# Deam0on/deepEMIA

Hardware: NVIDIA B200
Metric: instances_per_sec (higher is better)
Workload: dtype f32

## Files before the change

__graft_entry__.py:

```python
import os
import subprocess
import sys

ROOT = os.path.dirname(os.path.abspath(__file__))
CSRC = os.path.join(ROOT, "deepemia_b200", "csrc")
NVCC_FLAGS = ["-O3", "-lineinfo", "-fmad=false", "-std=c++17", "-gencode", "arch=compute_100a,code=sm_100a", "-shared",
              "-Xcompiler", "-fPIC"]


def _newer(target, sources):
    if not os.path.exists(target):
        return True
    t = os.path.getmtime(target)
    return any(os.path.getmtime(s) > t for s in sources)


def _sources():
    out = []
    for d, _, files in os.walk(CSRC):
        out += [os.path.join(d, f) for f in files if f.endswith((".cu", ".cuh", ".h"))]
    out.append(os.path.join(ROOT, "include", "emia.h"))
    return out


# ... 2 lines not shown
    if force or _newer(lib, _sources()):
        nvcc = os.environ.get("NVCC", "/usr/local/cuda/bin/nvcc")
        cmd = [nvcc] + NVCC_FLAGS + [os.path.join(CSRC, "emia_kernels.cu"), "-o", lib]
        subprocess.check_call(cmd, cwd=CSRC)
    hs_dir = os.path.join(ROOT, "tests", "hostsim")
    hs = os.path.join(hs_dir, "libemia_hostsim.so")
    if force or _newer(hs, _sources() + [os.path.join(hs_dir, "hostsim.cpp")]):
        subprocess.check_call(["g++", "-O2", "-ffp-contract=off", "-fPIC", "-shared", "-x", "c++", "hostsim.cpp", "-o", hs],
                              cwd=hs_dir)
    hs_rle = os.path.join(hs_dir, "libemia_hostsim_rle.so")
    if force or _newer(hs_rle, _sources() + [os.path.join(hs_dir, "hostsim_rle.cpp")]):
        subprocess.check_call(["g++", "-O2", "-ffp-contract=off", "-fPIC", "-shared", "-x", "c++", "hostsim_rle.cpp", "-o", hs_rle],
                              cwd=hs_dir)
    hs_text = os.path.join(hs_dir, "libemia_hostsim_text.so")
    if force or _newer(hs_text, _sources() + [os.path.join(hs_dir, "hostsim_text.cpp")]):
        subprocess.check_call(["g++", "-O2", "-ffp-contract=off", "-fPIC", "-shared", "-pthread", "-x", "c++", "hostsim_text.cpp", "-o",
                               hs_text], cwd=hs_dir)
    hs_shape = os.path.join(hs_dir, "libemia_hostsim_shape.so")
    if force or _newer(hs_shape, _sources() + [os.path.join(hs_dir, "hostsim_shape.cpp")]):
        subprocess.check_call(["g++", "-O2", "-ffp-contract=off", "-fPIC", "-shared", "-x", "c++", "hostsim_shape.cpp", "-o", hs_shape],
                              cwd=hs_dir)
    hs_nb = os.path.join(hs_dir, "libemia_hostsim_neighbour.so")
    if force or _newer(hs_nb, _sources() + [os.path.join(hs_dir, "hostsim_neighbour.cpp")]):
        subprocess.check_call(["g++", "-O2", "-ffp-contract=off", "-fPIC", "-shared", "-x", "c++", "hostsim_neighbour.cpp", "-o", hs_nb],
                              cwd=hs_dir)
    hs_trace = os.path.join(hs_dir, "libemia_hostsim_trace.so")
    if force or _newer(hs_trace, _sources() + [os.path.join(hs_dir, "hostsim_trace.cpp")]):
        subprocess.check_call(["g++", "-O2", "-ffp-contract=off", "-fPIC", "-shared", "-x", "c++", "hostsim_trace.cpp", "-o", hs_trace],
                              cwd=hs_dir)
    hs_coco = os.path.join(hs_dir, "libemia_hostsim_coco.so")
    if force or _newer(hs_coco, _sources() + [os.path.join(hs_dir, "hostsim_coco.cpp")]):
        subprocess.check_call(["g++", "-O2", "-ffp-contract=off", "-fPIC", "-shared", "-x", "c++", "hostsim_coco.cpp", "-o", hs_coco],
                              cwd=hs_dir)
    demo_dir = os.path.join(ROOT, "tests", "abi_demo")
    demo = os.path.join(demo_dir, "abi_demo")
    if force or _newer(demo, [os.path.join(demo_dir, "abi_demo.cpp"), os.path.join(ROOT, "include", "emia.h"), lib]):
        nvcc = os.environ.get("NVCC", "/usr/local/cuda/bin/nvcc")
        subprocess.check_call([nvcc, "-O2", "-std=c++17", "abi_demo.cpp", "-o", demo, "-L" + os.path.join(ROOT, "deepemia_b200"), "-lemia",
                               "-Xlinker", "-rpath", "-Xlinker", os.path.join("$ORIGIN", "..", "..", "deepemia_b200")], cwd=demo_dir)
    if ROOT not in sys.path:
        sys.path.insert(0, ROOT)
    import deepemia_b200
    from deepemia_b200 import _lib
    _lib.load()


def smoke():
    if ROOT not in sys.path:
        sys.path.insert(0, ROOT)
    import numpy as np
    import torch
    from deepemia_b200 import engine, synthetic as syn
    from oracle import pipeline
    dev = torch.device("cuda:0")
    H = W = 256
    probs, boxes, scores, classes = syn.synthetic_heads(42, 40, H, W, duplicate_frac=0.3, rmin=6, rmax=20, margin=20)
    t = [torch.as_tensor(a, device=dev) for a in (probs, boxes, scores, classes)]
    iset, kept, meas = engine.run_tiles(*t, [0, len(probs)], H, W, um_pix=0.5, rules=syn.POLYHIPES_RULES, frames=True)
    torch.cuda.synchronize()
    final, rows, _ = pipeline.run_tile(probs, boxes, scores, classes, H, W, um_pix=0.5, rules=syn.POLYHIPES_RULES)
    got = kept.to_lists()[0]
    assert got == final, (got, final)
    vals = [r[:12] for _, rr in meas.rows_to_host()[0] for r in rr if r[15] == 1.0]
    assert len(vals) == len(rows)
    for g, r in zip(vals, rows):
        np.testing.assert_allclose(g, np.array([float(v) for v in r[3:15]]), rtol=1e-5, atol=0)
# ... 8 lines not shown
```

deepemia_b200/_lib.py:

```python
import ctypes
import os

_HERE = os.path.dirname(os.path.abspath(__file__))
LIB_PATH = os.environ.get("EMIA_LIB_PATH") or os.path.join(_HERE, "libemia.so")

c_void_p, c_int, c_int64, c_float, c_double, c_size_t = (ctypes.c_void_p, ctypes.c_int, ctypes.c_int64, ctypes.c_float,
                                                         ctypes.c_double, ctypes.c_size_t)


class EmiaError(RuntimeError):
    pass


_SIGNATURES = {
    "emia_version": (c_int, []),
    "emia_last_error": (ctypes.c_char_p, []),
    "emia_scan_workspace_bytes": (c_size_t, [c_int64]),
    "emia_exclusive_scan_i64": (c_int, [c_void_p, c_int64, c_void_p, c_size_t, c_void_p]),
    "emia_paste_plan": (c_int, [c_void_p, c_int64, c_float, c_float, c_int, c_int, c_void_p, c_void_p, c_void_p]),
    "emia_paste_threshold_bitpack": (c_int, [c_void_p, c_void_p, c_void_p, c_void_p, c_int64, c_float, c_float, c_int, c_int,
                                             c_void_p, c_int64, c_int, c_void_p, c_void_p, c_void_p, c_int, c_void_p, c_void_p]),
    "emia_mask_bbox": (c_int, [c_void_p, c_int64, c_int, c_int, c_void_p, c_void_p, c_void_p, c_void_p, c_void_p]),
    "emia_mask_pack": (c_int, [c_void_p, c_int64, c_int, c_int, c_void_p, c_void_p, c_void_p, c_void_p]),
    "emia_mask_unpack": (c_int, [c_void_p, c_void_p, c_void_p, c_void_p, c_int64, c_int, c_int, c_void_p, c_void_p]),
    "emia_contour_count": (c_int, [c_void_p, c_void_p, c_void_p, c_int64, c_void_p, c_void_p, c_void_p, c_void_p, c_void_p]),
    "emia_contour_measure": (c_int, [c_void_p, c_void_p, c_void_p, c_int64, c_void_p, c_void_p, c_void_p, c_void_p, c_double,
                                     c_double, c_void_p, c_void_p, c_void_p, c_void_p, c_void_p, c_void_p, c_void_p]),
    "emia_contour_store": (c_int, [c_void_p, c_void_p, c_void_p, c_int64, c_void_p, c_void_p, c_void_p, c_void_p, c_void_p, c_void_p,
                                   c_void_p]),
    "emia_contour_trace_plan": (c_int, [c_void_p, c_int64, c_void_p, c_void_p]),
    "emia_contour_trace_slab": (c_int, [c_void_p, c_void_p, c_void_p, c_int64, c_void_p, c_void_p, c_int, c_void_p, c_void_p, c_void_p,
                                        c_void_p, c_void_p, c_void_p, c_void_p, c_void_p]),
    "emia_list_measure_plan": (c_int, [c_void_p, c_int, c_int, c_void_p, c_void_p, c_void_p, c_void_p, c_void_p, c_void_p, c_void_p,
                                       c_void_p]),
    "emia_contour_measure_list": (c_int, [c_int64, c_void_p, c_void_p, c_void_p, c_void_p, c_void_p, c_void_p, c_int, c_double, c_double,
                                          c_void_p, c_void_p, c_void_p, c_void_p, c_void_p, c_void_p, c_void_p]),
    "emia_list_measure_order": (c_int, [c_int64, c_void_p, c_void_p, c_void_p, c_void_p, c_int, c_void_p, c_void_p, c_void_p]),
    "emia_contour_shape_list": (c_int, [c_int64, c_void_p, c_void_p, c_void_p, c_void_p, c_void_p, c_void_p, c_int, c_double, c_void_p,
                                        c_void_p, c_void_p, c_void_p, c_void_p, c_void_p]),
    "emia_contour_measure_stored": (c_int, [c_void_p, c_int64, c_void_p, c_void_p, c_void_p, c_int, c_void_p, c_double, c_double,
                                            c_void_p, c_void_p, c_void_p, c_void_p, c_void_p, c_void_p]),
    "emia_group_workspace_bytes": (c_size_t, [c_void_p, c_int]),
    "emia_dedup_smart": (c_int, [c_void_p, c_void_p, c_void_p, c_void_p, c_void_p, c_void_p, c_void_p, c_void_p, c_void_p,
                                 c_void_p, c_int, c_int, c_int, c_void_p, c_void_p, c_double, c_double, c_void_p, c_void_p, c_void_p,
                                 c_size_t, c_void_p]),
    "emia_dedup_inorder": (c_int, [c_void_p, c_void_p, c_void_p, c_void_p, c_void_p, c_void_p, c_int, c_int, c_int, c_void_p, c_void_p,
                                   c_double, c_void_p, c_void_p, c_void_p, c_size_t, c_void_p]),
    "emia_dedup_sorted": (c_int, [c_void_p, c_void_p, c_void_p, c_void_p, c_void_p, c_void_p, c_void_p, c_int, c_int, c_int, c_void_p,
                                  c_void_p, c_double, c_void_p, c_void_p, c_void_p, c_size_t, c_void_p]),
    "emia_overlap_rules": (c_int, [c_void_p, c_void_p, c_void_p, c_void_p, c_void_p, c_void_p, c_void_p, c_void_p, c_int, c_int, c_int,
                                   c_void_p, c_void_p, c_void_p, c_void_p, c_int, c_void_p, c_void_p, c_void_p, c_size_t,
                                   c_void_p]),
    "emia_containment_rules": (c_int, [c_void_p, c_void_p, c_void_p, c_void_p, c_void_p, c_void_p, c_void_p, c_int, c_int, c_int,
                                       c_void_p, c_void_p, c_void_p, c_void_p, c_int, c_double, c_void_p, c_void_p, c_void_p,
# ... 103 lines not shown
```

deepemia_b200/csrc/core/emia_paste.cuh:

```cuda
#pragma once
#include "emia_common.cuh"

#define EMIA_MASK_SIDE 28

struct EmiaPasteBox {
    float x0, y0, x1, y1;
    int rx0, ry0, rx1, ry1;
    int valid;
};

EMIA_HD float emia_clampf(float v, float lo, float hi) { return v < lo ? lo : (v > hi ? hi : v); }

EMIA_HD EmiaPasteBox emia_paste_prepare(float bx0, float by0, float bx1, float by1, float scale_x, float scale_y, int W, int H) {
    EmiaPasteBox b;
    b.x0 = emia_clampf(bx0 * scale_x, 0.f, (float)W);
    b.x1 = emia_clampf(bx1 * scale_x, 0.f, (float)W);
    b.y0 = emia_clampf(by0 * scale_y, 0.f, (float)H);
    b.y1 = emia_clampf(by1 * scale_y, 0.f, (float)H);
    b.valid = ((b.x1 - b.x0) > 0.f) && ((b.y1 - b.y0) > 0.f);
    b.rx0 = emia_max((int)floorf(b.x0) - 1, 0);
    b.ry0 = emia_max((int)floorf(b.y0) - 1, 0);
    b.rx1 = emia_min((int)ceilf(b.x1) + 1, W);
    b.ry1 = emia_min((int)ceilf(b.y1) + 1, H);
    if (!b.valid) { b.rx0 = b.ry0 = b.rx1 = b.ry1 = 0; }
// ... 8 lines not shown

EMIA_HD EmiaAxisTap emia_paste_axis(int p, float lo, float hi) {
    const float c = (float)p + 0.5f;
    const float t = (c - lo) / (hi - lo);
    const float g = t * 2.f - 1.f;
    const float ix = emia_fmaf(g + 1.f, (float)EMIA_MASK_SIDE * 0.5f, -0.5f);
    const float fl = floorf(ix);
    EmiaAxisTap a;
    a.i0 = (int)fl;
    a.w1 = ix - fl;
    a.w0 = 1.f - a.w1;
    return a;
}

EMIA_HD float emia_paste_tap(const float* prob, int x, int y) {
    return ((unsigned)x < (unsigned)EMIA_MASK_SIDE && (unsigned)y < (unsigned)EMIA_MASK_SIDE) ? prob[y * EMIA_MASK_SIDE + x] : 0.f;
}

EMIA_HD float emia_paste_sample(const float* prob, const EmiaAxisTap& ax, const EmiaAxisTap& ay) {
    const float nw = ay.w0 * ax.w0;
    const float ne = ay.w0 * ax.w1;
    const float sw = ay.w1 * ax.w0;
    const float se = ay.w1 * ax.w1;
    const float v_nw = emia_paste_tap(prob, ax.i0, ay.i0);
    const float v_ne = emia_paste_tap(prob, ax.i0 + 1, ay.i0);
    const float v_sw = emia_paste_tap(prob, ax.i0, ay.i0 + 1);
    const float v_se = emia_paste_tap(prob, ax.i0 + 1, ay.i0 + 1);
    float acc = v_nw * nw;
    acc = emia_fmaf(v_ne, ne, acc);
    acc = emia_fmaf(v_sw, sw, acc);
    acc = emia_fmaf(v_se, se, acc);
    return acc;
}
```

deepemia_b200/csrc/emia_kernels.cu:

```cuda
#include <cuda_runtime.h>
#include <cuda_fp16.h>
#include <stdio.h>
#include <stdlib.h>
#include <string.h>
#include <algorithm>
#include <type_traits>
#include "../../include/emia.h"
#include "core/emia_common.cuh"
#include "core/emia_contour.cuh"
#include "core/emia_hull.cuh"
#include "core/emia_ellipse.cuh"
#include "core/emia_measure.cuh"
#include "core/emia_paste.cuh"
#include "core/emia_nms.cuh"
#include "core/emia_moments.cuh"
#include "core/emia_rle.cuh"
#include "core/emia_text.cuh"
#include "core/emia_shape.cuh"
#include "core/emia_neighbour.cuh"
#include "core/emia_coco.cuh"

static thread_local char g_err[512] = "";
static int emia_fail(int code, const char* fmt, const char* detail) {
    snprintf(g_err, sizeof(g_err), fmt, detail);
// ... 472 lines not shown
        }
        __syncthreads();
        (void)piece_rows_bytes;
    }
    if (tid == 0) asm volatile("cp.async.bulk.wait_group 0;" ::: "memory");
}

#define EMIA_P2_PAD_STRIDE 36
#define EMIA_P2_PAD_ROWS 32
#define EMIA_P2_BAND_ROWS 128
#define EMIA_P2_MAX_COLS 2112
#ifndef EMIA_P2_MIN_CTAS
#define EMIA_P2_MIN_CTAS 4
#endif

__device__ __forceinline__ void emia_st256_zero(void* p) {
    asm volatile("st.global.v4.b64 [%0], {%1, %1, %1, %1};" ::"l"(p), "l"(0ull) : "memory");
}
__device__ __forceinline__ void emia_st256(void* p, uint4 a, uint4 b) {
    asm volatile("st.global.v4.b64 [%0], {%1, %2, %3, %4};" ::"l"(p), "l"(((unsigned long long)a.y << 32) | a.x),
                 "l"(((unsigned long long)a.w << 32) | a.z), "l"(((unsigned long long)b.y << 32) | b.x),
                 "l"(((unsigned long long)b.w << 32) | b.z)
                 : "memory");
}
__device__ __forceinline__ void emia_cp_async16(void* sdst, const void* gsrc) {
    asm volatile("cp.async.cg.shared.global [%0], [%1], 16;" ::"r"((uint32_t)__cvta_generic_to_shared(sdst)), "l"(gsrc) : "memory");
}
__device__ __forceinline__ int emia_clampi(int v, int lo, int hi) { return v < lo ? lo : (v > hi ? hi : v); }

template <bool kHalf>
__global__ void __launch_bounds__(EMIA_PASTE_THREADS, EMIA_P2_MIN_CTAS) k_paste_v2(
    const void* __restrict__ probs_raw, const float4* __restrict__ boxes, const emia_inst_meta* __restrict__ meta,
    const int64_t* __restrict__ crop_off, int64_t n, float sx, float sy, int H, int W, uint32_t* __restrict__ frames,
    int64_t frame_slots, int pitch_words, uint32_t* __restrict__ crops, int32_t* __restrict__ bbox, int32_t* __restrict__ area,
    const int32_t* __restrict__ abort_flag) {
    if (abort_flag && *abort_flag) return;
    __shared__ __align__(16) float s_pp2[2][EMIA_P2_PAD_ROWS * EMIA_P2_PAD_STRIDE];
    __shared__ __align__(16) __half s_half2[2][kHalf ? EMIA_MASK_SIDE * EMIA_MASK_SIDE : 8];
    const float* probs = (const float*)probs_raw;
    const __half* probs_h = (const __half*)probs_raw;
    __shared__ __align__(32) uint32_t s_tile[EMIA_PASTE_TILE_WORDS];
    __shared__ int2 s_ctap[EMIA_P2_MAX_COLS];
    __shared__ int2 s_rtap[EMIA_P2_BAND_ROWS];
    __shared__ int s_red[5];

    const int tid = threadIdx.x;
    const int lane = tid & 31;
    const int warp = tid >> 5;
    const int nwarps = EMIA_PASTE_THREADS / 32;
    const int cpr = pitch_words >> 3;
    for (int k = tid; k < 2 * EMIA_P2_PAD_ROWS * EMIA_P2_PAD_STRIDE; k += EMIA_PASTE_THREADS) (&s_pp2[0][0])[k] = 0.f;
    __syncthreads();
    auto issue = [&](int64_t q, bool q_live, int b) {
        if (q_live) {
            if (kHalf) {
                if (tid < (EMIA_MASK_SIDE * EMIA_MASK_SIDE) / 8)
                    emia_cp_async16(&s_half2[b][tid * 8], probs_h + q * (EMIA_MASK_SIDE * EMIA_MASK_SIDE) + tid * 8);
            } else if (tid < EMIA_MASK_SIDE * 7) {
                const int r = tid / 7, c7 = tid - r * 7;
                emia_cp_async16(&s_pp2[b][(r + 2) * EMIA_P2_PAD_STRIDE + 4 + c7 * 4],
                                probs + q * (EMIA_MASK_SIDE * EMIA_MASK_SIDE) + r * EMIA_MASK_SIDE + c7 * 4);
            }
        }
        asm volatile("cp.async.commit_group;" ::: "memory");
    };
    emia_inst_meta m_next;
    float4 bx_next = make_float4(0.f, 0.f, 0.f, 0.f);
    m_next.valid = 0; m_next.ch = m_next.cw = 0;
    if ((int64_t)blockIdx.x < n) { m_next = meta[blockIdx.x]; bx_next = boxes[blockIdx.x]; }
    issue(blockIdx.x, (int64_t)blockIdx.x < n && m_next.valid && m_next.ch > 0 && m_next.cw > 0, 0);
    int buf = 0;

    for (int64_t inst = blockIdx.x; inst < n; inst += gridDim.x) {
        const emia_inst_meta m = m_next;
        const float4 bx = bx_next;
        float* s_pp = s_pp2[buf];
        const __half* s_half = s_half2[buf];
        const EmiaPasteBox pb = emia_paste_prepare(bx.x, bx.y, bx.z, bx.w, sx, sy, W, H);
        const bool live = m.valid && m.ch > 0 && m.cw > 0;
        if (tid < 5) s_red[tid] = (tid == 0) ? 0 : ((tid == 1 || tid == 2) ? 0x7fffffff : -1);
        const int cc0 = live ? (m.wc0 >> 3) : 0;
        const int cc1 = live ? ((m.wc0 + m.cw - 1) >> 3) : -1;
        unsigned char* frame = nullptr;
        if (frames) {
            frame = (unsigned char*)(frames + (size_t)(inst % frame_slots) * (size_t)H * (size_t)pitch_words);
            const int total = H * cpr;
            const int top = live ? m.ry0 * cpr : total;
            const int bot0 = live ? (m.ry0 + m.ch) * cpr : total;
            for (int q = tid; q < top; q += EMIA_PASTE_THREADS) emia_st256_zero(frame + (size_t)q * 32);
            for (int q = bot0 + tid; q < total; q += EMIA_PASTE_THREADS) emia_st256_zero(frame + (size_t)q * 32);
            if (live && cc1 - cc0 + 1 < cpr) {
                for (int r = tid; r < m.ch; r += EMIA_PASTE_THREADS) {
                    unsigned char* row = frame + (size_t)(m.ry0 + r) * cpr * 32;
                    for (int c = 0; c < cc0; ++c) emia_st256_zero(row + c * 32);
                    for (int c = cc1 + 1; c < cpr; ++c) emia_st256_zero(row + c * 32);
                }
            }
        }
        {
            const int64_t nx = inst + gridDim.x;
            bool nlive = false;
            if (nx < n) { m_next = meta[nx]; bx_next = boxes[nx]; nlive = m_next.valid && m_next.ch > 0 && m_next.cw > 0; }
            issue(nx, nlive, buf ^ 1);
        }
        if (live) {
            const int ncols = m.cw * 32;
            for (int k = tid; k < ncols; k += EMIA_PASTE_THREADS) {
                const int x = m.wc0 * 32 + k;
                const EmiaAxisTap a = emia_paste_axis(x, pb.x0, pb.x1);
                const int i0 = (x >= m.rx0 && x < m.rx1) ? emia_clampi(a.i0, -2, EMIA_MASK_SIDE) : -2;
                s_ctap[k] = make_int2(i0 + 4, __float_as_int(a.w1));
            }
        }
        asm volatile("cp.async.wait_group 1;" ::: "memory");
        __syncthreads();
        if (kHalf) {
            if (live)
                for (int k = tid; k < EMIA_MASK_SIDE * EMIA_MASK_SIDE; k += EMIA_PASTE_THREADS) {
                    const int r = k / EMIA_MASK_SIDE, c = k - r * EMIA_MASK_SIDE;
                    s_pp[(r + 2) * EMIA_P2_PAD_STRIDE + 4 + c] = __half2float(s_half[k]);
                }
            __syncthreads();
        }
        if (live) {
            const int span_chunks = cc1 - cc0 + 1;
            const int span_words = span_chunks * 8;
            const int woff = m.wc0 - cc0 * 8;
            const int rows_per_band = emia_min(EMIA_P2_BAND_ROWS, emia_max(1, EMIA_PASTE_TILE_WORDS / span_words));
// ... 15 lines not shown
                    const float xw0 = 1.f - xw1, yw0 = 1.f - yw1;
                    const float* t = &s_pp[rt.x + ct.x];
                    const float nw = yw0 * xw0;
                    const float ne = yw0 * xw1;
                    const float sw = yw1 * xw0;
                    const float se = yw1 * xw1;
                    float acc = t[0] * nw;
                    acc = emia_fmaf(t[1], ne, acc);
                    acc = emia_fmaf(t[EMIA_P2_PAD_STRIDE], sw, acc);
                    acc = emia_fmaf(t[EMIA_P2_PAD_STRIDE + 1], se, acc);
                    const uint32_t word = __ballot_sync(0xffffffffu, acc >= 0.5f);
                    if (lane == 0) s_tile[r * span_words + woff + c] = word;
                    r += step_r; c += step_c;
                    if (c >= m.cw) { c -= m.cw; ++r; }
                }
                __syncthreads();
                {
                    int rr = tid / m.cw, cc = tid - rr * m.cw;
                    const int sr = EMIA_PASTE_THREADS / m.cw, scw = EMIA_PASTE_THREADS - sr * m.cw;
                    while (rr < nr) {
                        const uint32_t word = s_tile[rr * span_words + woff + cc];
                        crop[(size_t)(r0 + rr) * m.cw + cc] = word;
                        if (word) {
                            const int y = m.ry0 + r0 + rr;
                            l_area += __popc(word);
                            l_ymin = min(l_ymin, y); l_ymax = max(l_ymax, y);
                            l_xmin = min(l_xmin, (m.wc0 + cc) * 32 + (__ffs((int)word) - 1));
                            l_xmax = max(l_xmax, (m.wc0 + cc) * 32 + (31 - __clz((int)word)));
                        }
                        rr += sr; cc += scw;
                        if (cc >= m.cw) { cc -= m.cw; ++rr; }
                    }
                }
                if (frames) {
                    const uint4* s4 = (const uint4*)s_tile;
                    int rr = tid / span_chunks, cc = tid - rr * span_chunks;
                    const int sr = EMIA_PASTE_THREADS / span_chunks, sc = EMIA_PASTE_THREADS - sr * span_chunks;
                    while (rr < nr) {
                        const int si = (rr * span_chunks + cc) * 2;
                        emia_st256(frame + ((size_t)(m.ry0 + r0 + rr) * cpr + cc0 + cc) * 32, s4[si], s4[si + 1]);
                        rr += sr; cc += sc;
                        if (cc >= span_chunks) { cc -= span_chunks; ++rr; }
                    }
                }
                __syncthreads();
            }
            for (int o = 16; o > 0; o >>= 1) {
                l_area += __shfl_xor_sync(0xffffffffu, l_area, o);
                l_ymin = min(l_ymin, __shfl_xor_sync(0xffffffffu, l_ymin, o)); l_xmin = min(l_xmin, __shfl_xor_sync(0xffffffffu, l_xmin, o));
                l_ymax = max(l_ymax, __shfl_xor_sync(0xffffffffu, l_ymax, o)); l_xmax = max(l_xmax, __shfl_xor_sync(0xffffffffu, l_xmax, o));
            }
            if (lane == 0 && l_area) {
                atomicAdd(&s_red[0], l_area);
                atomicMin(&s_red[1], l_ymin); atomicMin(&s_red[2], l_xmin);
                atomicMax(&s_red[3], l_ymax); atomicMax(&s_red[4], l_xmax);
            }
            __syncthreads();
        }
        if (tid == 0) {
            const int a = live ? s_red[0] : 0;
            area[inst] = a;
            ((int4*)bbox)[inst] = a > 0 ? make_int4(s_red[1], s_red[2], s_red[3], s_red[4]) : make_int4(-1, -1, -1, -1);
        }
        __syncthreads();
        buf ^= 1;
    }
    asm volatile("cp.async.wait_group 0;" ::: "memory");
}

extern "C" int emia_paste_threshold_bitpack(const float* probs, const float* boxes, const emia_inst_meta* meta,
                                            const int64_t* crop_off, int64_t n, float scale_x, float scale_y, int H,
                                            int W, uint32_t* frames, int64_t frame_slots, int pitch_words,
                                            uint32_t* crops, int32_t* bbox, int32_t* area, int variant_and_grid,
                                            const int32_t* abort_flag, void* stream) {
    const int variant = variant_and_grid & 0xff;
    const int ctas_req = (variant_and_grid >> 8) & 0xff;
    const bool probs_f16 = (variant_and_grid >> 16) & 1;
    if (n < 0 || H <= 0 || W <= 0) return emia_fail(EMIA_ERR_BAD_ARG, "emia_paste_threshold_bitpack: %s", "bad shape");
    if (n == 0) return EMIA_OK;
    if (!probs || !boxes || !meta || !crop_off || !crops || !bbox || !area)
        return emia_fail(EMIA_ERR_BAD_ARG, "emia_paste_threshold_bitpack: %s", "null pointer");
    if (frames) {
        if (pitch_words * 32 < W || (pitch_words & 3) || frame_slots <= 0)
            return emia_fail(EMIA_ERR_BAD_ARG, "emia_paste_threshold_bitpack: %s", "pitch_words must be a multiple of 4 covering W; frame_slots > 0");
        if (((uintptr_t)frames & 15) != 0) return emia_fail(EMIA_ERR_BAD_ARG, "emia_paste_threshold_bitpack: %s", "frames must be 16-byte aligned");
    }
    const int max_cols = ((W + 31) / 32 + 1) * 32;
    cudaStream_t st = (cudaStream_t)stream;
    const int sms = emia_num_sms();
    if (variant == 2 && max_cols <= EMIA_P2_MAX_COLS && ((uintptr_t)probs & 15) == 0 &&
        (!frames || ((pitch_words & 7) == 0 && ((uintptr_t)frames & 31) == 0))) {
        const int64_t per_sm = ctas_req ? ctas_req : 32;
        const unsigned grid = (unsigned)(n < (int64_t)sms * per_sm ? n : (int64_t)sms * per_sm);
        if (probs_f16)
            k_paste_v2<true><<<grid, EMIA_PASTE_THREADS, 0, st>>>(probs, (const float4*)boxes, meta, crop_off, n, scale_x, scale_y, H, W, frames,
                                                                  frames ? frame_slots : 1, pitch_words, crops, bbox, area, abort_flag);
        else
            k_paste_v2<false><<<grid, EMIA_PASTE_THREADS, 0, st>>>(probs, (const float4*)boxes, meta, crop_off, n, scale_x, scale_y, H, W, frames,
                                                                   frames ? frame_slots : 1, pitch_words, crops, bbox, area, abort_flag);
        return emia_check_launch("emia_paste_threshold_bitpack (v2) launch: %s");
    }
    if (probs_f16) return emia_fail(EMIA_ERR_UNSUPPORTED, "emia_paste_threshold_bitpack: %s", "fp16 probabilities need variant 2 (W <= 2048, 32-byte frame rows)");
    if (variant == 1 && frames) {
        if (pitch_words * 4 > EMIA_BULK_BYTES) return emia_fail(EMIA_ERR_UNSUPPORTED, "emia_paste_threshold_bitpack: %s", "variant 1 needs a frame row <= 16 KB");
        const size_t smem = 2 * EMIA_BULK_BYTES + EMIA_MASK_SIDE * EMIA_MASK_SIDE * 4 + (size_t)max_cols * 12;
        emia_need_dyn_smem((const void*)k_paste_bulk, smem);
        const int64_t per_sm = ctas_req ? ctas_req : 4;
        const unsigned grid = (unsigned)(n < (int64_t)sms * per_sm ? n : (int64_t)sms * per_sm);
        k_paste_bulk<<<grid, EMIA_PASTE_THREADS, smem, st>>>(probs, (const float4*)boxes, meta, crop_off, n, scale_x, scale_y, H, W,
                                                             frames, frame_slots, pitch_words, crops, bbox, area, max_cols, abort_flag);
        return emia_check_launch("emia_paste_threshold_bitpack (bulk) launch: %s");
    }
    const size_t smem = EMIA_MASK_SIDE * EMIA_MASK_SIDE * 4 + EMIA_PASTE_TILE_WORDS * 4 + (size_t)max_cols * 12;
    const int64_t per_sm = ctas_req ? ctas_req : 8;
    const unsigned grid = (unsigned)(n < (int64_t)sms * per_sm ? n : (int64_t)sms * per_sm);
    if (frames) {
        emia_need_dyn_smem((const void*)k_paste<true>, smem);
        k_paste<true><<<grid, EMIA_PASTE_THREADS, smem, st>>>(probs, (const float4*)boxes, meta, crop_off, n, scale_x, scale_y, H, W,
                                                              frames, frame_slots, pitch_words, crops, bbox, area, max_cols, abort_flag);
    } else {
        emia_need_dyn_smem((const void*)k_paste<false>, smem);
        k_paste<false><<<grid, EMIA_PASTE_THREADS, smem, st>>>(probs, (const float4*)boxes, meta, crop_off, n, scale_x, scale_y, H, W,
                                                               nullptr, 1, pitch_words, crops, bbox, area, max_cols, abort_flag);
    }
    return emia_check_launch("emia_paste_threshold_bitpack launch: %s");
}

#include "emia_masks.cuh"
#include "emia_morpho_kernels.cuh"
#include "emia_group_kernels.cuh"
#include "emia_morph_kernels.cuh"
#include "emia_tile_kernels.cuh"
#include "emia_rle_kernels.cuh"
#include "emia_text_kernels.cuh"
#include "emia_coco_kernels.cuh"
#include "emia_neighbour_kernels.cuh"
#include "emia_flow_kernels.cuh"
#include "emia_scalebar_kernels.cuh"
```

deepemia_b200/engine.py:

```python
import csv
import io
import math
from dataclasses import dataclass, field
from typing import Optional

import numpy as np
import torch

from . import _lib

MASK_SIDE = 28
REC_FIELDS = 16
(REC_MAJOR, REC_MINOR, REC_ECC, REC_LENGTH, REC_WIDTH, REC_CED, REC_ASPECT, REC_CIRC, REC_CHORDS, REC_FERET, REC_ROUND,
 REC_SPHER, REC_AREA, REC_PERIM, REC_NVERT, REC_MEASURED) = range(16)

FUSED_K4 = True
MEASURE_ORDER = bool(int(__import__("os").environ.get("EMIA_MEASURE_ORDER", "1")))
MEASURE_ORDER_MIN_SLOTS = 65536
LAUNCHES = {"count": 0}
STAGE_TIMING = {"enabled": False, "events": []}


NVTX = {"enabled": bool(int(__import__("os").environ.get("EMIA_NVTX", "0")))}


class _stage:

    def __init__(self, name):
        self.name = name

    def __enter__(self):
        if NVTX["enabled"]:
            torch.cuda.nvtx.range_push("emia:" + self.name)
        if STAGE_TIMING["enabled"]:
            self.a = torch.cuda.Event(enable_timing=True); self.b = torch.cuda.Event(enable_timing=True)
            self.a.record()
        return self

    def __exit__(self, *exc):
        if STAGE_TIMING["enabled"]:
            self.b.record()
            STAGE_TIMING["events"].append((self.name, self.a, self.b))
        if NVTX["enabled"]:
            torch.cuda.nvtx.range_pop()
        return False


def stage_summary():
    torch.cuda.synchronize()
# ... 109 lines not shown
    cont_off: Optional[torch.Tensor] = None
    pt_off: Optional[torch.Tensor] = None
    pts: Optional[torch.Tensor] = None
    cstart: Optional[torch.Tensor] = None
    records: Optional[torch.Tensor] = None
    rec_inst: Optional[torch.Tensor] = None
    perim0: Optional[torch.Tensor] = None
    n_records: int = 0
    cstart_stride: int = 0
    extra: dict = field(default_factory=dict)

    @property
    def device(self):
        return self.meta.device

    @property
    def valid(self):
        return self.meta[:, 6] != 0


def paste_plan(boxes, H, W, scale_x=1.0, scale_y=1.0):
    lib = _lib.load()
    n = int(boxes.shape[0])
    assert boxes.dtype == torch.float32 and boxes.is_contiguous()
    meta = torch.empty((n, 8), dtype=torch.int32, device=boxes.device)
    crop_off = torch.empty(n + 1, dtype=torch.int64, device=boxes.device)
    with _stage("paste_plan+scan"):
        _lib.check(lib.emia_paste_plan(_ptr(boxes), n, scale_x, scale_y, H, W, _ptr(meta), _ptr(crop_off), _stream()), "emia_paste_plan")
        exclusive_scan_(crop_off)
    LAUNCHES["count"] += 1
    return meta, crop_off


def paste(probs, boxes, H, W, scores=None, classes=None, scale_x=1.0, scale_y=1.0, frames=None, frame_slots=0,
          variant=2, crops_out=None, plan=None, ctas_per_sm=0, abort=None):
    lib = _lib.load()
    dev = probs.device
    n = int(probs.shape[0])
    assert probs.dtype in (torch.float32, torch.float16) and boxes.dtype == torch.float32 and probs.is_contiguous() and boxes.is_contiguous()
    st = _stream()
    if probs.dtype == torch.float16 and (variant != 2 or ((W + 31) // 32 + 1) * 32 > 2112):
        probs = probs.to(torch.float32)
    f16 = (1 << 16) if probs.dtype == torch.float16 else 0
    if plan is None:
        meta, crop_off = paste_plan(boxes, H, W, scale_x, scale_y)
        total = buffer_len(crop_off[n:], n)
    else:
        meta, crop_off, total = plan
        assert meta.shape[0] == n and crop_off.numel() == n + 1 and meta.is_contiguous() and crop_off.is_contiguous()
    if crops_out is not None:
        assert crops_out.numel() >= max(total, 1)
        crops = crops_out
    else:
        crops = torch.empty(max(total, 1), dtype=torch.int32, device=dev)
    bbox = torch.empty((n, 4), dtype=torch.int32, device=dev)
    area = torch.empty(n, dtype=torch.int32, device=dev)
    pw = pitch_words_for(W)
    if frames is True:
        frames = torch.empty((max(n, 1), H, pw), dtype=torch.int32, device=dev)
    slots = int(frames.shape[0]) if frames is not None else 1
    if frames is not None:
        assert frames.shape[1] == H and frames.shape[2] == pw and frames.is_contiguous()
    with _stage("k1_paste"):
        _lib.check(lib.emia_paste_threshold_bitpack(_ptr(probs), _ptr(boxes), _ptr(meta), _ptr(crop_off), n, scale_x, scale_y, H, W,
                                                    _ptr(frames), slots, pw, _ptr(crops), _ptr(bbox), _ptr(area),
                                                    int(variant) | (int(ctas_per_sm) << 8) | f16, _ptr(abort), st),
                   "emia_paste_threshold_bitpack")
    LAUNCHES["count"] += 1
    return InstanceSet(n=n, H=H, W=W, meta=meta, crop_off=crop_off, crops=crops, bbox=bbox, area=area, scores=scores,
                       classes=classes, frames=frames, total_crop_words=total)


def from_masks(masks, scores=None, classes=None):
    lib = _lib.load()
    dev = masks.device
    if masks.dtype == torch.bool:
        masks = masks.view(torch.uint8)
    assert masks.dtype == torch.uint8 and masks.is_contiguous() and masks.dim() == 3
    n, H, W = (int(s) for s in masks.shape)
    meta = torch.empty((n, 8), dtype=torch.int32, device=dev)
    crop_off = torch.empty(n + 1, dtype=torch.int64, device=dev)
    bbox = torch.empty((n, 4), dtype=torch.int32, device=dev)
    area = torch.empty(n, dtype=torch.int32, device=dev)
    st = _stream()
    _lib.check(lib.emia_mask_bbox(_ptr(masks), n, H, W, _ptr(meta), _ptr(crop_off), _ptr(bbox), _ptr(area), st), "emia_mask_bbox")
    exclusive_scan_(crop_off)
    total = buffer_len(crop_off[n:], n)
    crops = torch.empty(max(total, 1), dtype=torch.int32, device=dev)
    _lib.check(lib.emia_mask_pack(_ptr(masks), n, H, W, _ptr(meta), _ptr(crop_off), _ptr(crops), st), "emia_mask_pack")
    LAUNCHES["count"] += 2
    return InstanceSet(n=n, H=H, W=W, meta=meta, crop_off=crop_off, crops=crops, bbox=bbox, area=area, scores=scores,
                       classes=classes, total_crop_words=total)


def unpack_masks(iset, idx=None):
    lib = _lib.load()
    dev = iset.device
    if idx is None:
        k = iset.n
        idx_t = None
# ... 1547 lines not shown
```

include/emia.h:

```cpp
#ifndef EMIA_H
#define EMIA_H
#include <stddef.h>
#include <stdint.h>

#ifdef __cplusplus
extern "C" {
#endif

#define EMIA_OK 0
#define EMIA_ERR_BAD_ARG (-1)
#define EMIA_ERR_UNSUPPORTED (-2)
#define EMIA_ERR_LAUNCH (-3)
#define EMIA_ERR_WORKSPACE (-4)

#define EMIA_MASK_SIDE 28
#define EMIA_PASTE_PROBS_F16 (1 << 16)
#define EMIA_REC_FIELDS 16

typedef struct emia_inst_meta {
    int32_t ry0;
    int32_t wc0;
    int32_t ch;
    int32_t cw;
    int32_t rx0;
    int32_t rx1;
    int32_t valid;
    int32_t reserved;
} emia_inst_meta;

enum emia_rec_field {
    EMIA_REC_MAJOR_AXIS = 0, EMIA_REC_MINOR_AXIS = 1, EMIA_REC_ECCENTRICITY = 2, EMIA_REC_LENGTH = 3,
    EMIA_REC_WIDTH = 4, EMIA_REC_CIRCULAR_ED = 5, EMIA_REC_ASPECT = 6, EMIA_REC_CIRCULARITY = 7,
    EMIA_REC_CHORDS = 8, EMIA_REC_FERET = 9, EMIA_REC_ROUNDNESS = 10, EMIA_REC_SPHERICITY = 11,
    EMIA_REC_AREA = 12, EMIA_REC_PERIMETER = 13, EMIA_REC_NVERT = 14, EMIA_REC_MEASURED = 15
};

int emia_version(void);
const char* emia_last_error(void);

size_t emia_scan_workspace_bytes(int64_t n);
int emia_exclusive_scan_i64(int64_t* data, int64_t n, void* workspace, size_t workspace_bytes, void* stream);


int emia_paste_plan(const float* boxes, int64_t n, float scale_x, float scale_y, int H, int W,
                    emia_inst_meta* meta, int64_t* crop_words, void* stream);
int emia_paste_threshold_bitpack(const float* probs, const float* boxes, const emia_inst_meta* meta,
                                 const int64_t* crop_off, int64_t n, float scale_x, float scale_y, int H, int W,
                                 uint32_t* frames, int64_t frame_slots, int pitch_words, uint32_t* crops,
                                 int32_t* bbox, int32_t* area, int variant, const int32_t* abort_flag, void* stream);

int emia_mask_bbox(const uint8_t* masks, int64_t n, int H, int W, emia_inst_meta* meta, int64_t* crop_words,
                   int32_t* bbox, int32_t* area, void* stream);
int emia_mask_pack(const uint8_t* masks, int64_t n, int H, int W, const emia_inst_meta* meta,
                   const int64_t* crop_off, uint32_t* crops, void* stream);
int emia_mask_unpack(const uint32_t* crops, const emia_inst_meta* meta, const int64_t* crop_off,
                     const int32_t* idx, int64_t n_idx, int H, int W, uint8_t* masks_out, void* stream);

int emia_contour_count(const uint32_t* crops, const emia_inst_meta* meta, const int64_t* crop_off, int64_t n,
                       uint32_t* marks, int64_t* n_contours, int64_t* n_points, int64_t* scratch_bytes,
                       void* stream);
int emia_contour_measure(const uint32_t* crops, const emia_inst_meta* meta, const int64_t* crop_off, int64_t n,
                         uint32_t* marks, const int64_t* cont_off, const int64_t* pt_off,
                         const int64_t* scratch_off, double um_pix, double min_area, uint32_t* pts,
                         int32_t* cstart, double* records, int32_t* rec_inst, double* perim0, uint8_t* scratch,
                         void* stream);

int emia_contour_store(const uint32_t* crops, const emia_inst_meta* meta, const int64_t* crop_off, int64_t n,
                       uint32_t* marks, const int64_t* cont_off, const int64_t* pt_off, uint32_t* pts, int32_t* cstart,
                       double* perim0, void* stream);

int emia_contour_trace_plan(const emia_inst_meta* meta, int64_t n, int64_t* pt_cap, void* stream);
int emia_contour_trace_slab(const uint32_t* crops, const emia_inst_meta* meta, const int64_t* crop_off, int64_t n,
                            uint32_t* marks, const int64_t* pt_cap_off, int32_t cap_contours, uint32_t* pts,
                            int32_t* cstart_slab, int64_t* n_contours, int64_t* scratch_bytes, int32_t* overflow,
                            double* perim0 , const int32_t* abort_flag,
                            void* stream);
int emia_contour_measure_stored(const emia_inst_meta* meta, int64_t n, const int64_t* cont_off, const int64_t* pt_off,
                                const int32_t* cstart, int32_t cstart_stride, const int64_t* scratch_off, double um_pix,
                                double min_area, const uint32_t* pts, double* records, int32_t* rec_inst, double* perim0,
                                uint8_t* scratch, void* stream);

int emia_list_measure_plan(const int32_t* cap_off, int32_t G, int32_t total_cap, const int32_t* in_len,
// ... 194 lines not shown
```

Measured before the change: 38.02 million.

## Track per-slot dirty spans to clear only stale frame regions in paste

Adds a per-slot span table recording the row/chunk rectangle last written to each ring frame slot, so the paste kernel zeroes only the previously dirty region outside the new instance's box instead of the whole frame background. It also skips writing frames for instances that will be overwritten later in the ring (only the last frame_slots instances write). This cuts frame-clearing store traffic, at the cost of a span table that needs reset kernels and version tracking in Python, which are fragile under graph capture and external frame mutation.

```diff
diff --git a/__graft_entry__.py b/__graft_entry__.py
--- a/__graft_entry__.py
+++ b/__graft_entry__.py
@@ -58,6 +58,9 @@
     if force or _newer(hs_coco, _sources() + [os.path.join(hs_dir, "hostsim_coco.cpp")]):
         subprocess.check_call(["g++", "-O2", "-ffp-contract=off", "-fPIC", "-shared", "-x", "c++", "hostsim_coco.cpp", "-o", hs_coco],
                               cwd=hs_dir)
+    hs_spans = os.path.join(hs_dir, "libemia_hostsim_frame_spans.so")
+    if force or _newer(hs_spans, _sources() + [os.path.join(hs_dir, "hostsim_frame_spans.cpp")]):
+        subprocess.check_call(["g++", "-O2", "-fPIC", "-shared", "-x", "c++", "hostsim_frame_spans.cpp", "-o", hs_spans], cwd=hs_dir)
     demo_dir = os.path.join(ROOT, "tests", "abi_demo")
     demo = os.path.join(demo_dir, "abi_demo")
     if force or _newer(demo, [os.path.join(demo_dir, "abi_demo.cpp"), os.path.join(ROOT, "include", "emia.h"), lib]):
diff --git a/deepemia_b200/_lib.py b/deepemia_b200/_lib.py
--- a/deepemia_b200/_lib.py
+++ b/deepemia_b200/_lib.py
@@ -20,6 +20,10 @@
     "emia_paste_plan": (c_int, [c_void_p, c_int64, c_float, c_float, c_int, c_int, c_void_p, c_void_p, c_void_p]),
     "emia_paste_threshold_bitpack": (c_int, [c_void_p, c_void_p, c_void_p, c_void_p, c_int64, c_float, c_float, c_int, c_int,
                                              c_void_p, c_int64, c_int, c_void_p, c_void_p, c_void_p, c_int, c_void_p, c_void_p]),
+    "emia_paste_threshold_bitpack_ring": (c_int, [c_void_p, c_void_p, c_void_p, c_void_p, c_int64, c_float, c_float, c_int, c_int,
+                                                  c_void_p, c_int64, c_void_p, c_int, c_void_p, c_void_p, c_void_p, c_int, c_void_p,
+                                                  c_void_p]),
+    "emia_frame_spans_reset": (c_int, [c_void_p, c_int64, c_int, c_int, c_void_p]),
     "emia_mask_bbox": (c_int, [c_void_p, c_int64, c_int, c_int, c_void_p, c_void_p, c_void_p, c_void_p, c_void_p]),
     "emia_mask_pack": (c_int, [c_void_p, c_int64, c_int, c_int, c_void_p, c_void_p, c_void_p, c_void_p]),
     "emia_mask_unpack": (c_int, [c_void_p, c_void_p, c_void_p, c_void_p, c_int64, c_int, c_int, c_void_p, c_void_p]),
diff --git a/deepemia_b200/csrc/core/emia_paste.cuh b/deepemia_b200/csrc/core/emia_paste.cuh
--- a/deepemia_b200/csrc/core/emia_paste.cuh
+++ b/deepemia_b200/csrc/core/emia_paste.cuh
@@ -64,3 +64,35 @@
     acc = emia_fmaf(v_se, se, acc);
     return acc;
 }
+
+struct EmiaSpan {
+    int r0, r1, c0, c1;
+};
+
+EMIA_HD uint64_t emia_span_pack(EmiaSpan s) {
+    return (uint64_t)(uint16_t)s.r0 | ((uint64_t)(uint16_t)s.r1 << 16) | ((uint64_t)(uint16_t)s.c0 << 32) |
+           ((uint64_t)(uint16_t)s.c1 << 48);
+}
+EMIA_HD EmiaSpan emia_span_unpack(uint64_t v) {
+    EmiaSpan s;
+    s.r0 = (int)(v & 0xffff); s.r1 = (int)((v >> 16) & 0xffff);
+    s.c0 = (int)((v >> 32) & 0xffff); s.c1 = (int)(int16_t)(uint16_t)(v >> 48);
+    return s;
+}
+EMIA_HD EmiaSpan emia_span_full(int H, int chunks_per_row) { EmiaSpan s; s.r0 = 0; s.r1 = H; s.c0 = 0; s.c1 = chunks_per_row - 1; return s; }
+EMIA_HD EmiaSpan emia_span_empty() { EmiaSpan s; s.r0 = s.r1 = 0; s.c0 = 0; s.c1 = -1; return s; }
+
+struct EmiaSpanRowClear {
+    int a0, a1, b0, b1;
+};
+
+EMIA_HD EmiaSpanRowClear emia_span_row_clear(EmiaSpan old, EmiaSpan nw, int y) {
+    EmiaSpanRowClear z;
+    z.a0 = 0; z.a1 = -1; z.b0 = 0; z.b1 = -1;
+    if (y < old.r0 || y >= old.r1 || old.c0 > old.c1) return z;
+    z.a0 = old.c0;
+    if (y < nw.r0 || y >= nw.r1 || nw.c0 > nw.c1) { z.a1 = old.c1; return z; }
+    z.a1 = emia_min(old.c1, nw.c0 - 1);
+    z.b0 = emia_max(old.c0, nw.c1 + 1); z.b1 = old.c1;
+    return z;
+}
diff --git a/deepemia_b200/csrc/emia_kernels.cu b/deepemia_b200/csrc/emia_kernels.cu
--- a/deepemia_b200/csrc/emia_kernels.cu
+++ b/deepemia_b200/csrc/emia_kernels.cu
@@ -528,8 +528,8 @@
 __global__ void __launch_bounds__(EMIA_PASTE_THREADS, EMIA_P2_MIN_CTAS) k_paste_v2(
     const void* __restrict__ probs_raw, const float4* __restrict__ boxes, const emia_inst_meta* __restrict__ meta,
     const int64_t* __restrict__ crop_off, int64_t n, float sx, float sy, int H, int W, uint32_t* __restrict__ frames,
-    int64_t frame_slots, int pitch_words, uint32_t* __restrict__ crops, int32_t* __restrict__ bbox, int32_t* __restrict__ area,
-    const int32_t* __restrict__ abort_flag) {
+    int64_t frame_slots, uint64_t* __restrict__ spans, int pitch_words, uint32_t* __restrict__ crops, int32_t* __restrict__ bbox,
+    int32_t* __restrict__ area, const int32_t* __restrict__ abort_flag) {
     if (abort_flag && *abort_flag) return;
     __shared__ __align__(16) float s_pp2[2][EMIA_P2_PAD_ROWS * EMIA_P2_PAD_STRIDE];
     __shared__ __align__(16) __half s_half2[2][kHalf ? EMIA_MASK_SIDE * EMIA_MASK_SIDE : 8];
@@ -578,18 +578,31 @@
         const int cc0 = live ? (m.wc0 >> 3) : 0;
         const int cc1 = live ? ((m.wc0 + m.cw - 1) >> 3) : -1;
         unsigned char* frame = nullptr;
-        if (frames) {
-            frame = (unsigned char*)(frames + (size_t)(inst % frame_slots) * (size_t)H * (size_t)pitch_words);
-            const int total = H * cpr;
-            const int top = live ? m.ry0 * cpr : total;
-            const int bot0 = live ? (m.ry0 + m.ch) * cpr : total;
-            for (int q = tid; q < top; q += EMIA_PASTE_THREADS) emia_st256_zero(frame + (size_t)q * 32);
-            for (int q = bot0 + tid; q < total; q += EMIA_PASTE_THREADS) emia_st256_zero(frame + (size_t)q * 32);
-            if (live && cc1 - cc0 + 1 < cpr) {
-                for (int r = tid; r < m.ch; r += EMIA_PASTE_THREADS) {
-                    unsigned char* row = frame + (size_t)(m.ry0 + r) * cpr * 32;
-                    for (int c = 0; c < cc0; ++c) emia_st256_zero(row + c * 32);
-                    for (int c = cc1 + 1; c < cpr; ++c) emia_st256_zero(row + c * 32);
+        if (frames && inst + frame_slots >= n) {
+            const int64_t slot = inst % frame_slots;
+            frame = (unsigned char*)(frames + (size_t)slot * (size_t)H * (size_t)pitch_words);
+            if (spans) {
+                const EmiaSpan old = emia_span_unpack(spans[slot]);
+                EmiaSpan nw = emia_span_empty();
+                if (live) { nw.r0 = m.ry0; nw.r1 = m.ry0 + m.ch; nw.c0 = cc0; nw.c1 = cc1; }
+                for (int y = old.r0 + tid; y < old.r1; y += EMIA_PASTE_THREADS) {
+                    const EmiaSpanRowClear z = emia_span_row_clear(old, nw, y);
+                    unsigned char* row = frame + (size_t)y * cpr * 32;
+                    for (int c = z.a0; c <= z.a1; ++c) emia_st256_zero(row + c * 32);
+                    for (int c = z.b0; c <= z.b1; ++c) emia_st256_zero(row + c * 32);
+                }
+            } else {
+                const int total = H * cpr;
+                const int top = live ? m.ry0 * cpr : total;
+                const int bot0 = live ? (m.ry0 + m.ch) * cpr : total;
+                for (int q = tid; q < top; q += EMIA_PASTE_THREADS) emia_st256_zero(frame + (size_t)q * 32);
+                for (int q = bot0 + tid; q < total; q += EMIA_PASTE_THREADS) emia_st256_zero(frame + (size_t)q * 32);
+                if (live && cc1 - cc0 + 1 < cpr) {
+                    for (int r = tid; r < m.ch; r += EMIA_PASTE_THREADS) {
+                        unsigned char* row = frame + (size_t)(m.ry0 + r) * cpr * 32;
+                        for (int c = 0; c < cc0; ++c) emia_st256_zero(row + c * 32);
+                        for (int c = cc1 + 1; c < cpr; ++c) emia_st256_zero(row + c * 32);
+                    }
                 }
             }
         }
@@ -671,7 +684,7 @@
                         if (cc >= m.cw) { cc -= m.cw; ++rr; }
                     }
                 }
-                if (frames) {
+                if (frame) {
                     const uint4* s4 = (const uint4*)s_tile;
                     int rr = tid / span_chunks, cc = tid - rr * span_chunks;
                     const int sr = EMIA_PASTE_THREADS / span_chunks, sc = EMIA_PASTE_THREADS - sr * span_chunks;
@@ -700,6 +713,11 @@
             const int a = live ? s_red[0] : 0;
             area[inst] = a;
             ((int4*)bbox)[inst] = a > 0 ? make_int4(s_red[1], s_red[2], s_red[3], s_red[4]) : make_int4(-1, -1, -1, -1);
+            if (frame && spans) {
+                EmiaSpan nw = emia_span_empty();
+                if (live) { nw.r0 = m.ry0; nw.r1 = m.ry0 + m.ch; nw.c0 = cc0; nw.c1 = cc1; }
+                spans[inst % frame_slots] = emia_span_pack(nw);
+            }
         }
         __syncthreads();
         buf ^= 1;
@@ -707,11 +725,29 @@
     asm volatile("cp.async.wait_group 0;" ::: "memory");
 }
 
-extern "C" int emia_paste_threshold_bitpack(const float* probs, const float* boxes, const emia_inst_meta* meta,
-                                            const int64_t* crop_off, int64_t n, float scale_x, float scale_y, int H,
-                                            int W, uint32_t* frames, int64_t frame_slots, int pitch_words,
-                                            uint32_t* crops, int32_t* bbox, int32_t* area, int variant_and_grid,
-                                            const int32_t* abort_flag, void* stream) {
+__global__ void k_frame_spans_reset(uint64_t* __restrict__ spans, int64_t n, uint64_t full, const int32_t* __restrict__ abort_flag) {
+    if (abort_flag && *abort_flag) return;
+    for (int64_t i = (int64_t)blockIdx.x * blockDim.x + threadIdx.x; i < n; i += (int64_t)gridDim.x * blockDim.x) spans[i] = full;
+}
+
+static void emia_frame_spans_reset_launch(uint64_t* spans, int64_t n, int H, int pitch_words, const int32_t* abort_flag, cudaStream_t st) {
+    const int64_t blocks = (n + 255) / 256;
+    k_frame_spans_reset<<<(unsigned)(blocks < 4096 ? blocks : 4096), 256, 0, st>>>(
+        spans, n, emia_span_pack(emia_span_full(H, pitch_words >> 3)), abort_flag);
+}
+
+extern "C" int emia_frame_spans_reset(uint64_t* frame_spans, int64_t frame_slots, int H, int pitch_words, void* stream) {
+    if (!frame_spans || frame_slots <= 0 || H <= 0 || H > 0xffff || pitch_words <= 0 || (pitch_words & 7))
+        return emia_fail(EMIA_ERR_BAD_ARG, "emia_frame_spans_reset: %s", "bad argument");
+    emia_frame_spans_reset_launch(frame_spans, frame_slots, H, pitch_words, nullptr, (cudaStream_t)stream);
+    return emia_check_launch("emia_frame_spans_reset launch: %s");
+}
+
+extern "C" int emia_paste_threshold_bitpack_ring(const float* probs, const float* boxes, const emia_inst_meta* meta,
+                                                 const int64_t* crop_off, int64_t n, float scale_x, float scale_y, int H,
+                                                 int W, uint32_t* frames, int64_t frame_slots, uint64_t* frame_spans,
+                                                 int pitch_words, uint32_t* crops, int32_t* bbox, int32_t* area,
+                                                 int variant_and_grid, const int32_t* abort_flag, void* stream) {
     const int variant = variant_and_grid & 0xff;
     const int ctas_req = (variant_and_grid >> 8) & 0xff;
     const bool probs_f16 = (variant_and_grid >> 16) & 1;
@@ -723,7 +759,10 @@
         if (pitch_words * 32 < W || (pitch_words & 3) || frame_slots <= 0)
             return emia_fail(EMIA_ERR_BAD_ARG, "emia_paste_threshold_bitpack: %s", "pitch_words must be a multiple of 4 covering W; frame_slots > 0");
         if (((uintptr_t)frames & 15) != 0) return emia_fail(EMIA_ERR_BAD_ARG, "emia_paste_threshold_bitpack: %s", "frames must be 16-byte aligned");
-    }
+        if (frame_spans && (H > 0xffff || (pitch_words & 7)))
+            return emia_fail(EMIA_ERR_BAD_ARG, "emia_paste_threshold_bitpack_ring: %s", "a span table needs H <= 65535 and 32-byte frame rows");
+    }
+    if (!frames) frame_spans = nullptr;
     const int max_cols = ((W + 31) / 32 + 1) * 32;
     cudaStream_t st = (cudaStream_t)stream;
     const int sms = emia_num_sms();
@@ -733,10 +772,10 @@
         const unsigned grid = (unsigned)(n < (int64_t)sms * per_sm ? n : (int64_t)sms * per_sm);
         if (probs_f16)
             k_paste_v2<true><<<grid, EMIA_PASTE_THREADS, 0, st>>>(probs, (const float4*)boxes, meta, crop_off, n, scale_x, scale_y, H, W, frames,
-                                                                  frames ? frame_slots : 1, pitch_words, crops, bbox, area, abort_flag);
+                                                                  frames ? frame_slots : 1, frame_spans, pitch_words, crops, bbox, area, abort_flag);
         else
             k_paste_v2<false><<<grid, EMIA_PASTE_THREADS, 0, st>>>(probs, (const float4*)boxes, meta, crop_off, n, scale_x, scale_y, H, W, frames,
-                                                                   frames ? frame_slots : 1, pitch_words, crops, bbox, area, abort_flag);
+                                                                   frames ? frame_slots : 1, frame_spans, pitch_words, crops, bbox, area, abort_flag);
         return emia_check_launch("emia_paste_threshold_bitpack (v2) launch: %s");
     }
     if (probs_f16) return emia_fail(EMIA_ERR_UNSUPPORTED, "emia_paste_threshold_bitpack: %s", "fp16 probabilities need variant 2 (W <= 2048, 32-byte frame rows)");
@@ -748,6 +787,7 @@
         const unsigned grid = (unsigned)(n < (int64_t)sms * per_sm ? n : (int64_t)sms * per_sm);
         k_paste_bulk<<<grid, EMIA_PASTE_THREADS, smem, st>>>(probs, (const float4*)boxes, meta, crop_off, n, scale_x, scale_y, H, W,
                                                              frames, frame_slots, pitch_words, crops, bbox, area, max_cols, abort_flag);
+        if (frame_spans) emia_frame_spans_reset_launch(frame_spans, n < frame_slots ? n : frame_slots, H, pitch_words, abort_flag, st);
         return emia_check_launch("emia_paste_threshold_bitpack (bulk) launch: %s");
     }
     const size_t smem = EMIA_MASK_SIDE * EMIA_MASK_SIDE * 4 + EMIA_PASTE_TILE_WORDS * 4 + (size_t)max_cols * 12;
@@ -757,12 +797,22 @@
         emia_need_dyn_smem((const void*)k_paste<true>, smem);
         k_paste<true><<<grid, EMIA_PASTE_THREADS, smem, st>>>(probs, (const float4*)boxes, meta, crop_off, n, scale_x, scale_y, H, W,
                                                               frames, frame_slots, pitch_words, crops, bbox, area, max_cols, abort_flag);
+        if (frame_spans) emia_frame_spans_reset_launch(frame_spans, n < frame_slots ? n : frame_slots, H, pitch_words, abort_flag, st);
     } else {
         emia_need_dyn_smem((const void*)k_paste<false>, smem);
         k_paste<false><<<grid, EMIA_PASTE_THREADS, smem, st>>>(probs, (const float4*)boxes, meta, crop_off, n, scale_x, scale_y, H, W,
                                                                nullptr, 1, pitch_words, crops, bbox, area, max_cols, abort_flag);
     }
     return emia_check_launch("emia_paste_threshold_bitpack launch: %s");
+}
+
+extern "C" int emia_paste_threshold_bitpack(const float* probs, const float* boxes, const emia_inst_meta* meta,
+                                            const int64_t* crop_off, int64_t n, float scale_x, float scale_y, int H,
+                                            int W, uint32_t* frames, int64_t frame_slots, int pitch_words,
+                                            uint32_t* crops, int32_t* bbox, int32_t* area, int variant_and_grid,
+                                            const int32_t* abort_flag, void* stream) {
+    return emia_paste_threshold_bitpack_ring(probs, boxes, meta, crop_off, n, scale_x, scale_y, H, W, frames, frame_slots, nullptr,
+                                             pitch_words, crops, bbox, area, variant_and_grid, abort_flag, stream);
 }
 
 #include "emia_masks.cuh"
diff --git a/deepemia_b200/engine.py b/deepemia_b200/engine.py
--- a/deepemia_b200/engine.py
+++ b/deepemia_b200/engine.py
@@ -1,6 +1,7 @@
 import csv
 import io
 import math
+import weakref
 from dataclasses import dataclass, field
 from typing import Optional
 
@@ -15,6 +16,7 @@
  REC_SPHER, REC_AREA, REC_PERIM, REC_NVERT, REC_MEASURED) = range(16)
 
 FUSED_K4 = True
+FRAME_SPANS = True
 MEASURE_ORDER = bool(int(__import__("os").environ.get("EMIA_MEASURE_ORDER", "1")))
 MEASURE_ORDER_MIN_SLOTS = 65536
 LAUNCHES = {"count": 0}
@@ -190,6 +192,43 @@
     return meta, crop_off
 
 
+_FRAME_SPANS = {}
+
+
+def _frame_spans(frames, H, pw):
+    base = frames if frames._base is None else frames._base
+    key = id(base)
+    ent = _FRAME_SPANS.get(key)
+    capturing = torch.cuda.is_current_stream_capturing()
+    whole = frames.storage_offset() == 0 and frames.numel() * frames.element_size() == frames.untyped_storage().nbytes()
+    if not (FRAME_SPANS and whole and H <= 0xffff):
+        if ent is not None and ent[0] is not None:
+            ent[1] = None
+            if capturing:
+                ent[0] = None
+        return None
+    lib = _lib.load()
+    geom = (int(frames.shape[0]), H, pw)
+    if ent is None or (ent[0] is not None and ent[2] != geom):
+        if ent is None:
+            weakref.finalize(base, _FRAME_SPANS.pop, key, None)
+        if capturing:
+            _FRAME_SPANS[key] = ent = [None, None, geom]
+            return None
+        ent = [torch.empty(geom[0], dtype=torch.int64, device=frames.device), None, geom]
+        _FRAME_SPANS[key] = ent
+    if ent[0] is None:
+        return None
+    if ent[1] != frames._version:
+        if capturing:
+            ent[0] = None
+            return None
+        _lib.check(lib.emia_frame_spans_reset(_ptr(ent[0]), geom[0], H, pw, _stream()), "emia_frame_spans_reset")
+        LAUNCHES["count"] += 1
+        ent[1] = frames._version
+    return ent[0]
+
+
 def paste(probs, boxes, H, W, scores=None, classes=None, scale_x=1.0, scale_y=1.0, frames=None, frame_slots=0,
           variant=2, crops_out=None, plan=None, ctas_per_sm=0, abort=None):
     lib = _lib.load()
@@ -214,16 +253,18 @@
     bbox = torch.empty((n, 4), dtype=torch.int32, device=dev)
     area = torch.empty(n, dtype=torch.int32, device=dev)
     pw = pitch_words_for(W)
+    spans = None
     if frames is True:
         frames = torch.empty((max(n, 1), H, pw), dtype=torch.int32, device=dev)
+    elif frames is not None:
+        assert frames.shape[1] == H and frames.shape[2] == pw and frames.is_contiguous()
+        spans = _frame_spans(frames, H, pw)
     slots = int(frames.shape[0]) if frames is not None else 1
-    if frames is not None:
-        assert frames.shape[1] == H and frames.shape[2] == pw and frames.is_contiguous()
     with _stage("k1_paste"):
-        _lib.check(lib.emia_paste_threshold_bitpack(_ptr(probs), _ptr(boxes), _ptr(meta), _ptr(crop_off), n, scale_x, scale_y, H, W,
-                                                    _ptr(frames), slots, pw, _ptr(crops), _ptr(bbox), _ptr(area),
-                                                    int(variant) | (int(ctas_per_sm) << 8) | f16, _ptr(abort), st),
-                   "emia_paste_threshold_bitpack")
+        _lib.check(lib.emia_paste_threshold_bitpack_ring(_ptr(probs), _ptr(boxes), _ptr(meta), _ptr(crop_off), n, scale_x, scale_y, H,
+                                                         W, _ptr(frames), slots, _ptr(spans), pw, _ptr(crops), _ptr(bbox), _ptr(area),
+                                                         int(variant) | (int(ctas_per_sm) << 8) | f16, _ptr(abort), st),
+                   "emia_paste_threshold_bitpack_ring")
     LAUNCHES["count"] += 1
     return InstanceSet(n=n, H=H, W=W, meta=meta, crop_off=crop_off, crops=crops, bbox=bbox, area=area, scores=scores,
                        classes=classes, frames=frames, total_crop_words=total)
diff --git a/include/emia.h b/include/emia.h
--- a/include/emia.h
+++ b/include/emia.h
@@ -48,6 +48,12 @@
                                  const int64_t* crop_off, int64_t n, float scale_x, float scale_y, int H, int W,
                                  uint32_t* frames, int64_t frame_slots, int pitch_words, uint32_t* crops,
                                  int32_t* bbox, int32_t* area, int variant, const int32_t* abort_flag, void* stream);
+int emia_paste_threshold_bitpack_ring(const float* probs, const float* boxes, const emia_inst_meta* meta,
+                                      const int64_t* crop_off, int64_t n, float scale_x, float scale_y, int H, int W,
+                                      uint32_t* frames, int64_t frame_slots, uint64_t* frame_spans, int pitch_words,
+                                      uint32_t* crops, int32_t* bbox, int32_t* area, int variant, const int32_t* abort_flag,
+                                      void* stream);
+int emia_frame_spans_reset(uint64_t* frame_spans, int64_t frame_slots, int H, int pitch_words, void* stream);
 
 int emia_mask_bbox(const uint8_t* masks, int64_t n, int H, int W, emia_inst_meta* meta, int64_t* crop_words,
                    int32_t* bbox, int32_t* area, void* stream);
```

After: 78.36 million (median of 6 runs). +106.1%, better.
